# HJReachability/ilqgames

Measured on AMD Instinct MI355X. Metric: iLQ iterations/sec (batch), higher is better.
Workload: dtype f64

## Files before the change

### ilqgames_amd/csrc/ilqg_api.hip

```cpp
#include <hip/hip_runtime.h>

#include <cstdio>
#include <cstdlib>
#include <cmath>
#include <chrono>
#include <cstring>
#include <string>
#include <vector>

#include "ilqg_common.hpp"
#include "ilqg_lq.hpp"
#include "ilqg_lq_openloop.hpp"
#include "ilqg_lq_feedback2.hpp"
#include "ilqg_lq_generic.hpp"
#include "ilqg_costates.hpp"
#include "ilqg_models.hpp"
#include "ilqg_nash.hpp"
#include "ilqg_receding.hpp"
#include "ilqg_rowprog.hpp"
#include "ilqg_rowprog_static.hpp"
#include "ilqg_solve.hpp"
#include "ilqg_stages.hpp"

using namespace ilqg;
// ... 1366 lines not shown
  }
  const bool counted = !opt.forced_steps && (split || !(fixed_iters > 0 && !al_mode) || choice(opt.counted, false));
  const bool handoff = counted && !split && !kProfile && sa.prm.linesearch && choice(opt.handoff, true);
  const bool lists = split || handoff;
  sa.defer_forward = (!split && !open_loop) ? 1 : 0;
  {
    constexpr size_t fwd_elems = 4 * 2 * ((NX * NX + C::SCR + 3) & ~3) + 2 * NX + 8;
    if (trial_rows_elems(d, sa.rows_cw, static_prog != 0) < fwd_elems + 8) sa.defer_forward = 0;
  }
  const bool adjoint = choice(opt.adjoint_expected_decrease, sa.defer_forward == 0);
  const bool single_wave = has_1w && pw && sa.compact && !kProfile && (adjoint || sa.defer_forward) &&
                           d.rp_compact_w <= W1Cfg<T, NX, NP, MU>::kWords &&
                           choice(opt.single_wave_sweep, !opt.deterministic && size_t(sched_batch) >= size_t(5) * num_cus);
  if (single_wave) {
    sa.prio_div = 0;
    if (adjoint) sa.defer_forward = 0;
  }
  constexpr bool has_packed = sizeof(T) == 4 && C::USE_MFMA && C::MFMA_ONE_TILE && NP == 3;
  bool b_const = false;
  if (open_loop) {
    plan.sweep = {ol_compact ? ilq_lq_kernel<T, NX, NP, MU, LQ_OPEN_LOOP_COMPACT> : ilq_lq_kernel<T, NX, NP, MU, LQ_OPEN_LOOP>,
                  O::NT, (O::LDS_ELEMS + 4) * sizeof(T)};
  } else if constexpr (!C::USE_MFMA) {
    plan.sweep = {ilq_lq_kernel<T, NX, NP, MU, LQ_VALU_FEEDBACK>, C::NT, C::LDS_ELEMS * sizeof(T)};
  } else {
    plan.sweep = {ilq_lq_kernel<T, NX, NP, MU, LQ_PLAYER_WAVES>, 64 * NP,
                  (MfmaSweepLds<T, NX, NP, MU>::ELEMS + (C::MFMA_ONE_TILE ? 0 : 4)) * sizeof(T)};
    constexpr bool has_forms = C::MFMA_ONE_TILE && SolveRows<NP * MU, NX + 1>::FITS;
    const bool forms = choice(opt.sweep_forms, true);
    constexpr bool has_bconst = has_forms && NX < 16 && MU == 2;
    b_const = has_bconst && forms && p->b_constant && sa.compact && sa.defer_forward && !single_wave;
    if constexpr (has_forms)
      if (!forms) plan.sweep.kernel = ilq_lq_kernel<T, NX, NP, MU, LQ_PLAYER_WAVES, 0>;
    if constexpr (has_bconst)
      if (b_const) plan.sweep.kernel = ilq_lq_kernel<T, NX, NP, MU, LQ_PLAYER_WAVES, 2>;
    if constexpr (has_packed) {
      if (size_t(sched_batch) >= size_t(5) * 256) {
        plan.sweep.kernel = ilq_lq_kernel<T, NX, NP, MU, LQ_PLAYER_WAVES_PACKED>;
        if constexpr (has_forms)
          if (!forms) plan.sweep.kernel = ilq_lq_kernel<T, NX, NP, MU, LQ_PLAYER_WAVES_PACKED, 0>;
        if constexpr (has_bconst)
          if (b_const) plan.sweep.kernel = ilq_lq_kernel<T, NX, NP, MU, LQ_PLAYER_WAVES_PACKED, 2>;
      }
    }
    if constexpr (has_1w) {
      if (single_wave) {
        plan.sweep = {ilq_lq_kernel<T, NX, NP, MU, LQ_SINGLE_WAVE>, 64, size_t(W1Cfg<T, NX, NP, MU>::ELEMS + 4) * sizeof(T)};
        if constexpr (has_forms)
          if (!forms) plan.sweep.kernel = ilq_lq_kernel<T, NX, NP, MU, LQ_SINGLE_WAVE, 0>;
      }
    }
  }
  sa.clear_counters = 1;
  plan.trial = {k_trial, 64 * W, lds_trial};
  plan.exit = {ilq_exit_kernel<T, NX, NP, MU>, nt_exit, quad_tables_bytes(d, sizeof(T)) + 64 * sizeof(T)};
  plan.read_restarts = counted && al_mode;
  constexpr bool pairs = rollout_pairs(NX, NP, MU);
  if (lists) {
    const size_t lds_roll = trial_phase_lds_bytes<T>(d, TRIAL_ROLL, sa.rows_cw);
    const size_t lds_proll = pairs ? size_t(rollout_pair_lds_elems(d.n, d.m)) * sizeof(T) + 16 : lds_roll;
    const size_t static_regs_lds = (rows_state_in_registers(NX, NP * MU) ? 0 : size_t(d.n + d.m) * 64) * sizeof(T) + 16;
    const int rows_cw = static_id ? 64 : sa.rows_cw;
    const bool regs = static_id && static_in_regs;
    plan.roll = {ilq_roll_kernel<T, NX, NP, MU>, 64, lds_proll};
    plan.rows = {k_rows, 64, regs ? static_regs_lds : split_maps_bytes + split_rows_elems(d, NX, rows_cw) * sizeof(T)};
    plan.decide = {d.inst_solver ? ilq_decide_kernel<T, NX, NP, MU, true> : ilq_decide_kernel<T, NX, NP, MU, false>, 64,
                   trial_phase_lds_bytes<T>(d, TRIAL_DECIDE, sa.rows_cw)};
    plan.prows = {k_prows, 64, regs ? static_regs_lds : split_maps_bytes + probe_rows_elems(d, NX, rows_cw) * sizeof(T)};
    plan.proll = {ilq_probe_roll_kernel<T, NX, NP, MU>, 64, lds_proll};
    plan.proll_fat = {ilq_probe_roll_kernel<T, NX, NP, MU, sizeof(T) == 8>, 64, lds_proll};
    if (pairs) {
      plan.proll_single = {ilq_probe_roll_kernel<T, NX, NP, MU, sizeof(T) == 8, true>, 64, lds_roll};
      plan.proll_lanes = {ilq_probe_roll_lanes_kernel<T, NX, NP, MU>, 64, size_t(rollout_lanes_lds_elems(d.n, d.m, d.N)) * sizeof(T) + 16};
    }
  }
  plan.cap = al_mode ? (long long)(sa.prm.max_solver_iters + 1) * (sa.prm.unconstrained_solver_max_iters + 2)
                     : (long long)sa.prm.max_solver_iters + 2;
  if (split || counted) plan.cap = (plan.cap + 2) * ((long long)sa.prm.max_backtracking_steps + 3);
  plan.row_chunks = (d.T + sa.rows_cw - 1) / sa.rows_cw;
  plan.lane_width = rollout_lanes_per_wave(NP > 0 ? NP : 1);
  plan.num_cus = num_cus;
  plan.split = split; plan.counted = counted; plan.handoff = handoff; plan.lists = lists; plan.pairs = pairs;
  plan.timed = opt.max_runtime > 0.0 && counted;
  plan.bursts = counted && !kProfile && !plan.timed && choice(opt.round_bursts, true);
  plan.probe = lists && sa.prm.linesearch && choice(opt.probe, true);
  plan.lanes_auto = NX <= 16;
  plan.deep_tails = true;
  p->last_schedule = (single_wave ? ILQG_SCHEDULE_SINGLE_WAVE_SWEEP : 0) | ((single_wave && adjoint) ? ILQG_SCHEDULE_ADJOINT_DECREASE : 0) |
                     (split ? ILQG_SCHEDULE_SPLIT_TRIAL : 0) | (sa.compact ? ILQG_SCHEDULE_COMPACT_ROWS : 0) |
                     (counted ? ILQG_SCHEDULE_COUNTED : 0) | (open_loop ? ILQG_SCHEDULE_OPEN_LOOP : 0) |
                     ((static_prog || (static_id && split)) ? ILQG_SCHEDULE_STATIC_ROWS : 0) |
                     (b_const ? ILQG_SCHEDULE_CONSTANT_B : 0);
  return run_rounds(p, sa, tail, plan, opt, stream);
}

#if defined(ILQG_PART_NX)
template struct DimsLaunch<float, ILQG_PART_NX, ILQG_PART_NP, ILQG_PART_MU>;
template struct DimsLaunch<double, ILQG_PART_NX, ILQG_PART_NP, ILQG_PART_MU>;
#else
#if defined(ILQG_SPLIT_BUILD)
#define X(NX_, NP_, MU_)                                   \
  extern template struct DimsLaunch<float, NX_, NP_, MU_>; \
  extern template struct DimsLaunch<double, NX_, NP_, MU_>;
ILQG_FOR_DIMS(X)
#undef X
#endif

// ... 1020 lines not shown
```

### ilqgames_amd/csrc/ilqg_rows.hpp

```cpp
#pragma once

#include <type_traits>
#include <utility>

#include "ilqg_common.hpp"
#include "ilqg_models.hpp"

#ifndef ILQG_ROWS_XREG
#define ILQG_ROWS_XREG 1
#endif
#ifndef ILQG_PROFILE2
#define ILQG_PROFILE2 0
#endif

namespace ilqg {

#pragma clang fp contract(off)

typedef const __attribute__((address_space(4))) int* rp_cptr;
template <typename T> struct ConstPtr;
template <> struct ConstPtr<float> { typedef const __attribute__((address_space(4))) float* type; };
template <> struct ConstPtr<double> { typedef const __attribute__((address_space(4))) double* type; };

enum {
// ... 410 lines not shown
    if constexpr (BOUND && (F == RO_WEIGHT || F == RO_VALUE) && (mode == ROP_TERM || mode == ROP_EXT_EVAL || mode == ROP_EXT_APPLY || mode == ROP_JACOBIAN)) {
      const int c = cols[F == RO_WEIGHT ? 0 : 1];
      if (c >= 0 && iv) return iv[c];
    }
    return rt[F];
  }
  __device__ __forceinline__ SidsStatic<S, OP> sids() const { return SidsStatic<S, OP>{}; }
};
struct PassDynamic {
  int op_begin, op_end, reg_begin, reg_end, li_begin, li_count, pkind, player, li_grad;
};
template <class S, int PS>
struct PassStatic {
  static constexpr int b = S::w[RP_OFF_PASS] + PS * RPASS_WORDS;
  static constexpr int op_begin = S::w[b + 0], op_end = S::w[b + 1], reg_begin = S::w[b + 2], reg_end = S::w[b + 3],
                       li_begin = S::w[b + 4], li_count = S::w[b + 5], pkind = S::w[b + 6], player = S::w[b + 7],
                       li_grad = S::w[b + 8];
};

template <class S>
constexpr bool static_prog_in_registers() {
  const int nops = (S::w[RP_OFF_SIDS] - S::w[RP_OFF_OPS]) / ROP_WORDS;
  for (int op = 0; op < nops; op++) {
    const int b = S::w[RP_OFF_OPS] + op * ROP_WORDS;
    if (S::w[b + RO_MODE] == ROP_AFFINE || S::w[b + RO_NSID] > ROP_INLINE_SIDS) return false;
  }
  return S::w[RP_NUM_PSLOTS] + S::w[RP_MAX_LSLOTS] <= 64 && S::w[S::w[RP_OFF_COMPACT] + RC_W] > 0;
}
template <class S>
constexpr unsigned static_prog_pass_split() {
  const int np = S::w[RP_NUM_PASSES];
  int wgt[32] = {0};
  for (int ps = 0; ps < np && ps < 32; ps++) {
    const int b = S::w[RP_OFF_PASS] + ps * RPASS_WORDS;
    wgt[ps] = S::w[b + 1] - S::w[b + 0];
  }
  unsigned first = 0, taken = 0;
  int wa = 0, wb = 0;
  for (int k = 0; k < np && k < 32; k++) {
    int best = -1;
    for (int ps = 0; ps < np && ps < 32; ps++)
      if (!((taken >> ps) & 1u) && (best < 0 || wgt[ps] > wgt[best])) best = ps;
    taken |= 1u << best;
    if (wa <= wb) { first |= 1u << best; wa += wgt[best]; } else { wb += wgt[best]; }
  }
  return first;
}
template <class PROG, bool ST = PROG::STATIC> struct ProgInRegisters { static constexpr bool value = false; static constexpr int slots = 1; };
template <class PROG> struct ProgInRegisters<PROG, true> {
  static constexpr bool value = static_prog_in_registers<typename PROG::S>();
  static constexpr int slots = value ? PROG::S::w[RP_NUM_PSLOTS] + PROG::S::w[RP_MAX_LSLOTS] : 1;
};

template <typename T, int CN_, int CM_, int CNP_, bool XREG = false, bool GRAD_ONLY = false, class PROG = ProgDynamic>
__device__ __forceinline__ void rows_chunk(const DevProblem& p, const short* maps, const QuadArgs<T>& a, int k0,
                                           int nrows, int cw, T* sm, int lane, unsigned pass_mask = ~0u) {
  constexpr bool RT = CN_ == 0;
  constexpr bool ST = PROG::STATIC;
  static_assert(!XREG || (CN_ > 0 && CN_ <= 16 && CM_ <= 16), "register-held rows: compile-time n, m <= 16");
  const int CN = RT ? p.n : CN_, CM = RT ? p.m : CM_, CNP = RT ? p.N : CNP_;
  const int NA = CN + CM;
  constexpr bool REGACC = ProgInRegisters<PROG>::value;
  const int cws = REGACC ? 1 : (ST ? kStaticRowStride : cw + 1);
  const int ast = ST ? 64 : cw;
  T* const arg = sm;
  T* const acc = sm + (XREG ? 0 : NA) * ast;
  typedef typename std::conditional<XREG, MixArg<T>, RowArg<T>>::type Arg;
  const rp_cptr rp = (rp_cptr)p.row_prog;
  const rp_cptr iv = (rp_cptr) reinterpret_cast<const int*>(a.iv);
  const typename ConstPtr<T>::type segs =
      (typename ConstPtr<T>::type)(PROG::kBound ? problem_segs<T>(p) + a.seg_off : problem_segs<T>(p));
  auto hdr = [&](auto f) -> int {
    if constexpr (ST) { constexpr int v = PROG::S::w[decltype(f)::value]; return v; } else return rp[decltype(f)::value];
  };
#define ILQG_RP_HDR(F) hdr(std::integral_constant<int, F>{})
  const int num_passes = ILQG_RP_HDR(RP_NUM_PASSES), NPS = ILQG_RP_HDR(RP_NUM_PSLOTS);
  const rp_cptr passes = rp + ILQG_RP_HDR(RP_OFF_PASS);
  const rp_cptr ops = rp + ILQG_RP_HDR(RP_OFF_OPS);
  const rp_cptr sids = rp + ILQG_RP_HDR(RP_OFF_SIDS);
  const rp_cptr pinit = rp + ILQG_RP_HDR(RP_OFF_PINIT);
  const rp_cptr linit = rp + ILQG_RP_HDR(RP_OFF_LINIT);
  const rp_cptr regions = rp + ILQG_RP_HDR(RP_OFF_REGIONS);
  const rp_cptr merit = rp + ILQG_RP_HDR(RP_OFF_MERIT);
  const bool quad_out = !GRAD_ONLY && (a.Q != nullptr || (a.compact != nullptr && a.compact_quad));
  const bool do_quad = quad_out || a.merit_part != nullptr;
  const bool want_cost = !GRAD_ONLY && a.cost_part != nullptr;
  const PairTable& pt = p.pairs;
  long long qc0 = (kProfile && a.phacc) ? clock64() : 0, qc1;
#define ILQG_QPH(i) do { if (kProfile && a.phacc) { __builtin_amdgcn_sched_barrier(0); qc1 = clock64(); __builtin_amdgcn_sched_barrier(0); a.phacc[i] += qc1 - qc0; qc0 = qc1; } } while (0)

  {
    auto stage_rows = [&](const T* g, int dim, int first) {
      constexpr int UN = 8;
      const int total = cw * dim;
      for (int i0 = 0; i0 < total; i0 += 64 * UN) {
        T v[UN];
        int dst[UN];
#pragma unroll
        for (int u = 0; u < UN; u++) {
          const int i = i0 + u * 64 + lane;
          const bool in = i < total;
          const int ic = in ? i : 0;
          const int r = ic / dim, e = ic - r * dim;
          const int rs = r < nrows ? r : nrows - 1;
          dst[u] = in ? (first + e) * ast + r : -1;
          v[u] = g[rs * dim + e];
        }
// ... 184 lines not shown
        term_compute_leaf<T, Arg, true>(QuadTables<T>{}, c, v, lambda, a.mu, &o, &cc, tnom);
#if ILQG_PROFILE2
        ILQG_QPH(3);
#endif
        bool act = deriv && o.pattern != PAT_NONE;
        if (mode == ROP_EXT_EVAL) {
          const bool is_min = c.flags & ILQG_FLAG_IS_MIN;
          if (aux == 0 || (is_min && o.value < ext_value) || (!is_min && o.value > ext_value)) {
            ext_value = o.value;
            ext_best = aux;
          }
          return;
        }
        if (mode == ROP_EXT_APPLY) {
          if (aux == 0 && is_cost && live) ctot += ext_value;
          act = act && ext_best == aux;
        } else if (is_cost && live) {
          ctot += o.value;
        }
        if (act) {
          if (sid_inline)
            rows_scatter<T>(od.template field<RO_PATTERN_NSEG>(), o, sid, nsid, col, cws, v, quad_out);
          else
            rows_scatter<T>(od.template field<RO_PATTERN_NSEG>(), o, SidsTable{sids + od.template field<RO_SID>()}, nsid, col, cws, v, quad_out);
        }
#if ILQG_PROFILE2
        ILQG_QPH(4);
#endif
      };
      if constexpr (ST) {
        static_for<PD::op_begin, PD::op_end>([&](auto opc) {
          constexpr int OP = decltype(opc)::value;
          run_op(OpStatic<typename PROG::S, OP, PROG::kBound>{ops + OP * ROP_WORDS, iv, rp + (PROG::S::w[RP_WORDS] + OP * 2)});
        });
      } else {
        static_assert(ROP_WORDS <= 64, "an op descriptor is one word per lane");
        const int* const opsv = reinterpret_cast<const int*>(p.row_prog) + rp[RP_OFF_OPS];
        int next_words = (lane < ROP_WORDS && op_begin < op_end) ? opsv[op_begin * ROP_WORDS + lane] : 0;
#pragma unroll 1
        for (int op = op_begin; op < op_end; op++) {
          int words = next_words;
          if (op + 1 < op_end) next_words = lane < ROP_WORDS ? opsv[(op + 1) * ROP_WORDS + lane] : 0;
          if (iv) {
            const rp_cptr icols = rp + rp[RP_WORDS];
            const int wcol = icols[2 * op], vcol = icols[2 * op + 1];
            if (wcol >= 0) words = lane == RO_WEIGHT ? iv[wcol] : words;
            if (vcol >= 0) words = lane == RO_VALUE ? iv[vcol] : words;
          }
          run_op(OpDynamic{words});
        }
      }
      if (pkind == RPASS_PLAYER && valid) {
        if (want_cost) a.cost_part[size_t(row) * CNP + player] = ctot;
        if (a.merit_part) {
          T s1 = T(0), s2 = T(0);
          if constexpr (ST) {
            typedef typename PROG::S S;
            constexpr int mb = S::w[RP_OFF_MERIT] + PD::player * RMERIT_WORDS, sb = S::w[RP_OFF_SIDS];
            static_for<0, S::w[mb + 3]>([&](auto dc) {
              const T rv = col[S::w[sb + S::w[mb + 2] + decltype(dc)::value] * cws];
              s1 += rv * rv;
            });
            static_for<0, S::w[mb + 1]>([&](auto dc) {
              const T lv = col[S::w[sb + S::w[mb + 0] + decltype(dc)::value] * cws];
              s2 += lv * lv;
            });
          } else {
            const rp_cptr md = merit + player * RMERIT_WORDS;
            const rp_cptr ls = sids + md[0];
            const rp_cptr rs = sids + md[2];
            const int lcnt = md[1], rcnt = md[3];
            for (int d = 0; d < rcnt; d++) {
              const T rv = col[rs[d] * cws];
              s1 += rv * rv;
            }
            for (int d = 0; d < lcnt; d++) {
              const T lv = col[ls[d] * cws];
              s2 += lv * lv;
            }
          }
          a.merit_part[(size_t(row) * CNP + player) * 2 + 0] = s1;
          a.merit_part[(size_t(row) * CNP + player) * 2 + 1] = s2;
        }
      }
    }
    lds_sync(true);
    tl_stamp(a.tl, a.tl_b, 42 + 2 * (ps < 4 ? ps : 4), lane == 0);
#if !ILQG_PROFILE2
    if (pkind == RPASS_JACOBIANS) ILQG_QPH(1); else ILQG_QPH(2);
#else
    ILQG_QPH(0);
#endif
    if constexpr (!REGACC)
    for (int rg = reg_begin; rg < (GRAD_ONLY ? reg_begin : reg_end); rg++) {
      const rp_cptr rd = regions + rg * RREG_WORDS;
      const int arr = rd[0], words = rd[1], offs = rd[2];
      const short* const map = maps + rd[3];
      if (arr == RA_A) {
        if (a.A) {
          if constexpr (RT) rows_writeout_rt<T>(a.A + size_t(k0) * CN * CN, size_t(CN) * CN, CN * CN, map, acc, cws, nrows, lane);
          else rows_writeout<T, CN_ * CN_, rows_vec_width<T>(CN_ * CN_)>(a.A + size_t(k0) * CN * CN, CN * CN, map, acc, cws, nrows, lane);
        }
      } else if (arr == RA_B) {
        if (a.Bm) {
          if constexpr (RT) rows_writeout_rt<T>(a.Bm + size_t(k0) * CN * CM, size_t(CN) * CM, CN * CM, map, acc, cws, nrows, lane);
          else rows_writeout<T, CN_ * CM_, rows_vec_width<T>(CN_ * CM_)>(a.Bm + size_t(k0) * CN * CM, CN * CM, map, acc, cws, nrows, lane);
        }
      } else if (arr == RA_Q) {
        if (a.Q) {
          if constexpr (RT) rows_writeout_rt<T>(a.Q + size_t(k0) * CNP * CN * CN + offs, size_t(CNP) * CN * CN, CN * CN, map, acc, cws, nrows, lane);
          else rows_writeout<T, CN_ * CN_, rows_vec_width<T>(CN_ * CN_)>(a.Q + size_t(k0) * CNP * CN * CN + offs, size_t(CNP) * CN * CN, map, acc, cws, nrows, lane);
        }
      } else if (arr == RA_L) {
        if (a.l) rows_writeout_small<T>(a.l + size_t(k0) * CNP * CN + offs, CNP * CN, words, map, acc, cws, nrows, lane);
      } else if (arr == RA_R) {
        if (a.R) rows_writeout_small<T>(a.R + size_t(k0) * pt.Rsz + offs, pt.Rsz, words, map, acc, cws, nrows, lane);
      } else {
        if (a.r) rows_writeout_small<T>(a.r + size_t(k0) * pt.rsz + offs, pt.rsz, words, map, acc, cws, nrows, lane);
      }
    }
    if (!GRAD_ONLY && a.compact && (pkind == RPASS_PLAYER ? a.compact_quad : a.compact_lin)) {
      int CWD, base;
      if constexpr (ST) {
        typedef typename PROG::S S;
        constexpr int cbo = S::w[RP_OFF_COMPACT];
        CWD = S::w[cbo + RC_W];
        base = S::w[cbo + RC_BASE + (PD::pkind == RPASS_PLAYER ? 1 + PD::player : 0)];
      } else {
        const rp_cptr cb = rp + rp[RP_OFF_COMPACT];
        CWD = cb[RC_W];
        base = cb[RC_BASE + (pkind == RPASS_PLAYER ? 1 + player : 0)];
      }
      T* const g0 = a.compact + size_t(k0) * CWD + base;
      constexpr int RB = 8;
      if constexpr (REGACC) {
// ... 72 lines not shown
```

### ilqgames_amd/csrc/ilqg_solve.hpp

```cpp
#pragma once
#ifndef ILQG_ROLL_PRIO
#define ILQG_ROLL_PRIO 1
#endif

#include "ilqg_lq.hpp"
#include "ilqg_lq_openloop.hpp"
#include "ilqg_lq_feedback2.hpp"
#include "ilqg_lq_feedback1w.hpp"
#include "ilqg_lq_generic.hpp"
#include "ilqg_stages.hpp"

namespace ilqg {

template <typename T>
struct SolveArgs {
  const T* x0;
  T *xs, *us;
  T *P, *alpha;
  T* total_costs;
  int *iters, *status, *converged;
  const int* active;
  T* ws;
  size_t ws_stride;
  int fixed_iters;
  int batch;
  int ol_row;
  int al_mode;
  ilqg_solver_params prm;
  long long* prof;
  int first;
  int* unfinished;
  const int* ids;
  int* ids_next;
  int round_count;
  const T* forced_steps;
  int defer_forward;
  int prio_div;
  int compact;
  int rows_cw;
  T* probe_pool;
  int probe_k;
  int outer_closed;
  int clear_counters;
};


enum { ST_ROLLOUT = 0, ST_QUAD = 1, ST_LQ = 2, ST_INNER_DONE = 3, ST_DONE = 4, ST_PROBE = 5 };
enum { Q_COSTS = 0, Q_INIT = 1, Q_TRIAL = 2, Q_LIN = 3 };
template <typename T>
struct SolveState {
  int stage, qmode, initial, cur, sacc, num_iterations, bt, accepted_iters;
  int has_converged, ok, logged, inner_calls, al_success;
  int ed_pending;
  int rejected;
  int pad2;
  T acc_scale, step, last_merit, expected_decrease, max_err, mu;
};
constexpr int kStateElems = 32;
static_assert(sizeof(SolveState<float>) <= kStateElems * sizeof(float), "state slot");
static_assert(sizeof(SolveState<double>) <= kStateElems * sizeof(double), "state slot");

struct WsLayout {
  size_t xs1, us1, P1, al1, A, B, Q, l, R, r, lqscr, dx, mpart, cpart, ints, state, lambdas, wxs, wus, wP, wal, total;
  __host__ __device__ WsLayout(int n, int m, int N, int T, int Rsz, int rsz, int ol_row = 0, int num_constraints = 0,
                               int al_mode = 0) {
    size_t o = 0;
    auto take = [&](size_t cnt) {
      const size_t at = o;
      o += (cnt + 3) & ~size_t(3);
      return at;
    };
    xs1 = take(size_t(T) * n);
    us1 = take(size_t(T) * m);
    P1 = take(size_t(T) * m * n);
    al1 = take(size_t(T) * m);
    A = take(size_t(T) * n * n);
    B = take(size_t(T) * n * m);
    Q = take(size_t(T) * N * n * n);
    l = take(size_t(T) * N * n);
    R = take(size_t(T) * Rsz);
    r = take(size_t(T) * rsz);
    lqscr = take(size_t(T) * (size_t(ol_row) > size_t(N * (n + 1) + n) ? size_t(ol_row) : size_t(N * (n + 1) + n)));
    dx = take(size_t(T) * n);
    mpart = take(size_t(T) * N * 2);
    cpart = take(size_t(T) * N);
    ints = take(2 * kMaxPlayers);
    state = take(kStateElems);
    lambdas = take(size_t(num_constraints) * T);
    wxs = take(al_mode ? size_t(T) * n : 0);
    wus = take(al_mode ? size_t(T) * m : 0);
    wP = take(al_mode ? size_t(T) * m * n : 0);
    wal = take(al_mode ? size_t(T) * m : 0);
    total = o;
  }
};

// ... 544 lines not shown

template <typename T>
__device__ __forceinline__ void trial_rollout_args(const SolveArgs<T>& sa, const InstanceBuffers<T>& ib, int b, int n,
                                                   SolveState<T>& s, RolloutArgs<T>& ra) {
  const int snew = 1 - s.sacc;
  ra.x0 = s.initial ? sa.x0 + size_t(b) * n : ib.XS(s.cur);
  ra.xs_ref = s.initial ? ib.XS(0) : ib.XS(s.cur);
  ra.us_ref = s.initial ? ib.US(0) : ib.US(s.cur);
  ra.P = s.initial ? ib.PB(0) : ib.PB(snew);
  ra.alpha = s.initial ? ib.AL(0) : ib.AL(snew);
  ra.alpha_scale = s.initial ? T(1) : s.step;
  ra.xs = s.initial ? ib.XS(1) : ib.XS(1 - s.cur);
  ra.us = s.initial ? ib.US(1) : ib.US(1 - s.cur);
  if (s.initial) {
    s.cur = 1;
    s.qmode = Q_COSTS;
  } else {
    s.qmode = sa.prm.linesearch ? Q_TRIAL : Q_LIN;
  }
}

template <typename T, int NX, int NP, int MU>
__device__ __forceinline__ void roll_pair_instances(const DevProblem& p, const SolveArgs<T>& sa, int b0, int b1, T* sm) {
  constexpr int n = NX, N = NP, m = NP * MU;
  const InstanceBuffers<T> ib0(p, sa, b0), ib1(p, sa, b1 < 0 ? b0 : b1);
  SolveState<T> s0, s1;
  RolloutArgs<T> r0, r1;
  auto enter = [&](const InstanceBuffers<T>& ib, int b, SolveState<T>& s, RolloutArgs<T>& r) -> bool {
    if (b < 0) return false;
    if (!sa.first) {
      if (reinterpret_cast<const SolveState<T>*>(ib.w + ib.L.state)->stage != ST_ROLLOUT) return false;
    } else if (sa.active && !sa.active[b]) {
      if (threadIdx.x == 0) reinterpret_cast<SolveState<T>*>(ib.w + ib.L.state)->stage = ST_DONE;
      return false;
    }
    s = trial_state_begin<T>(p, sa, ib, b, n, N, m);
    if (s.stage != ST_ROLLOUT) return false;
    trial_rollout_args<T>(sa, ib, b, n, s, r);
    r.iv = instance_values(p, b);
    return true;
  };
  const bool g0 = enter(ib0, b0, s0, r0), g1 = enter(ib1, b1, s1, r1);
  if (!g0 && !g1) return;
  __syncthreads();
  rollout_pair<T, NX, NP * MU, (MU == 1)>(p, g0 ? r0 : r1, g1 ? r1 : r0, g0, g1, sm, int(threadIdx.x));
  if (g0) state_store<T>(ib0.w, ib0.L, s0);
  if (g1) state_store<T>(ib1.w, ib1.L, s1);
}

__host__ __device__ constexpr bool fused_rollout_room(int elem_bytes, int nx, int np, int mu, int progid) {
  return elem_bytes == 4 || (progid != 0 && nx == 14 && np == 3 && mu == 2);
}

template <typename T, int NX, int NP, int MU, int W, int PHASE = TRIAL_FUSED, int PROGID = 0, bool BOUND = (PROGID >= kBoundProg),
          bool SOLVER_COLS = true>
__device__ __forceinline__ void trial_part_instance(const DevProblem& p, const short* maps,
                                                    const SolveArgs<T>& sa, int b, T* sm) {
  static_assert(PHASE == TRIAL_FUSED || W == 1, "the split phases run one wave per instance");
  static_assert(NX > 0 || PHASE != TRIAL_FUSED, "the run-time-dimensioned path (NX = 0) runs the split passes");
  const int n = NX > 0 ? NX : p.n, N = NX > 0 ? NP : p.N, m = NX > 0 ? NP * MU : p.m;
  const int Tn = p.T;
  const InstanceBuffers<T> ib(p, sa, b);
  const WsLayout& L = ib.L;
  T* const w = ib.w;
  int* const t_extreme = ib.t_extreme();
  T* const lambdas = w + L.lambdas;
  T* const costs = sa.total_costs + size_t(b) * N;
  const int t = threadIdx.x, wave = t >> 6, lane = t & 63;

  const size_t re = PHASE == TRIAL_DECIDE ? 0 : (rollout_lds_elems(n, m) + 3) & ~size_t(3);
  const size_t qe = trial_phase_quad_elems<T>(p, PHASE, sa.rows_cw, PROGID != 0 && PHASE == TRIAL_FUSED);
  constexpr int RW = W > 1 ? W - 1 : 1;
  const int rwave = W > 1 ? wave - 1 : 0;
  T* const sm_roll = sm;
  T* const sm_quad = sm + re + size_t(rwave < 0 ? 0 : rwave) * qe;
  T* const sm_quad0 = sm + re;
  int* const flags = reinterpret_cast<int*>(sm + re + size_t(RW) * qe);
  T* const ed_slot = reinterpret_cast<T*>(flags + 2);

  SolveState<T> s = trial_state_begin<T>(p, sa, ib, b, n, N, m);
  tl_stamp(sa.prof, b, 0, t == 0);
  const long long pr_start = clock64();
  long long qph[8] = {0, 0, 0, 0, 0, 0, 0, 0};
  long long rph[4] = {0, 0, 0, 0};

#pragma unroll 1
  while (s.stage == ST_ROLLOUT || s.stage == ST_QUAD) {
    __syncthreads();
    const bool roll = PHASE != TRIAL_DECIDE && s.stage == ST_ROLLOUT;
    RolloutArgs<T> ra;
    if (roll) {
      trial_rollout_args<T>(sa, ib, b, n, s, ra);
      if constexpr (BOUND || PHASE == TRIAL_ROLL) ra.iv = instance_values(p, b);
    }
    if (t == 0) {
      flags[0] = roll ? 0 : Tn;
      flags[1] = 0;
    }
    __syncthreads();
    tl_stamp(sa.prof, b, 1, t == 0);
    if (roll && wave == 0) {
#if ILQG_ROLL_PRIO
      __builtin_amdgcn_s_setprio(ILQG_ROLL_PRIO);
#endif
      if constexpr (NX > 0)
        rollout_instance<T, NX, NP * MU, (NX == 4 && NP == 2), (MU == 1), (NX == 3 && NP == 2 && MU == 1),
                         (NX == 4 * NP && MU == 2 && NP <= 2), dims_use_plain_rk4(NX, NP, MU),
                         fused_rollout_room(int(sizeof(T)), NX, NP, MU, PROGID)>(
                                         p, ra, sm_roll, lane, W > 1 ? &flags[0] : nullptr,
                                         (kProfile && sa.prof) ? rph : nullptr, kTimeline ? sa.prof : nullptr, b);
      else
        rollout_instance_rt<T>(p, ra, sm_roll, lane);
#if ILQG_ROLL_PRIO
      __builtin_amdgcn_s_setprio(0);
#endif
    }
    tl_stamp(sa.prof, b, 2, t == 0);
    if (roll && W == 1) {
      __syncthreads();
      if (t == 0) flags[0] = Tn;
      __syncthreads();
    }
    if (PHASE == TRIAL_ROLL) break;

    const int qmode = s.qmode;
    if constexpr (PHASE == TRIAL_FUSED) {
    QuadArgs<T> qa = trial_quad_args<T, BOUND>(p, ib, s, sa.compact != 0, b);
    qa.phacc = (kProfile && sa.prof) ? qph : nullptr;
    qa.tl = kTimeline ? sa.prof : nullptr;
    qa.tl_b = b;
    long long tq0 = (kProfile && sa.prof) ? clock64() : 0;
    static_assert(W <= 2, "the deferred forward pass reads the linearisation on the first row wave while no other row wave "
                          "may overwrite it yet: with more than one row wave set defer_forward = 0 or hold them back");
    if (s.ed_pending && rwave == 0) {
      LQArgs<T> fa{};
      fa.A = w + L.A;
      fa.scratch = w + L.lqscr;
      fa.x0 = nullptr;
      fa.dx = nullptr;
      fa.ed_out = ed_slot;
      fa.T_steps = Tn;
      if (sa.compact) {
        fa.compact = w + L.Q;
        fa.compact_tab = p.row_prog + p.rp_compact_off;
        fa.dt = p.dt;
      }
      constexpr int FWD_LDSE = 4 * 2 * ((NX * NX + LQCfg<T, NX, NP, MU>::SCR + 3) & ~3) + 2 * NX + 8;
      lq_forward_pass_body<T, NX, NP, MU, 64, FWD_LDSE>(fa, sm_quad, lane);
    }
    tl_stamp(sa.prof, b, 3, rwave == 0 && lane == 0);
    typedef typename RowProgSel<PROGID>::type RowProg;
    constexpr bool SHARE_LAST = PROGID != 0 && W == 2 && ProgInRegisters<RowProg>::value && rows_state_in_registers(NX, NP * MU);
    if constexpr (SHARE_LAST) {
      const int cw = sa.rows_cw;
      const int nchunks = (Tn + cw - 1) / cw;
      const int rem = Tn % cw;
      constexpr unsigned first_half = static_prog_pass_split<typename RowProg::S>();
      if (wave == 0) qa.tl = nullptr;
#pragma unroll 1
      for (int c = (wave == 0 ? nchunks - 1 : 0); c < nchunks; c++) {
        const int k0 = rem == 0 ? c * cw : (c == 0 ? 0 : rem + (c - 1) * cw);
        const int nrows = (rem != 0 && c == 0) ? rem : cw;
        if (wave != 0)
          while (progress_observe(&flags[0]) < k0 + nrows) __builtin_amdgcn_s_sleep(8);
        tl_stamp(sa.prof, b, 4 + 2 * (c < 3 ? c : 3), wave != 0 && lane == 0);
        const unsigned mask = c == nchunks - 1 ? (wave == 0 ? first_half : ~first_half) : ~0u;
        rows_chunk<T, NX, NP * MU, NP, true, false, RowProg>(p, maps, qa, k0, nrows, cw, sm_quad, lane, mask);
        tl_stamp(sa.prof, b, 5 + 2 * (c < 3 ? c : 3), wave != 0 && lane == 0);
      }
    } else
    if (rwave >= 0) {
      const int cw = sa.rows_cw;
      const int nchunks = (Tn + cw - 1) / cw;
      auto claim = [&]() {
        int c = 0;
        if (lane == 0) c = atomicAdd(&flags[1], 1);
        return __builtin_amdgcn_readfirstlane(c);
      };
      const int rem = Tn % cw;
#pragma unroll 1
      for (int c = claim(); c < nchunks; c = claim()) {
        const int k0 = rem == 0 ? c * cw : (c == 0 ? 0 : rem + (c - 1) * cw);
        const int nrows = (rem != 0 && c == 0) ? rem : cw;
        while (progress_observe(&flags[0]) < k0 + nrows) __builtin_amdgcn_s_sleep(8);
        if (kProfile && sa.prof) { const long long tq1 = clock64(); qph[6] += tq1 - tq0; }
        tl_stamp(sa.prof, b, 4 + 2 * (c < 3 ? c : 3), lane == 0);
        rows_chunk<T, NX, NP * MU, NP, (PROGID != 0 && rows_state_in_registers(NX, NP * MU)), false, typename RowProgSel<PROGID>::type>(
            p, maps, qa, k0, nrows, cw, sm_quad, lane);
        tl_stamp(sa.prof, b, 5 + 2 * (c < 3 ? c : 3), lane == 0);
        if (kProfile && sa.prof) { tq0 = clock64(); qph[7] += 1; }
      }
    }
    }

    if (PHASE == TRIAL_FUSED && s.ed_pending) {
      __syncthreads();
      s.expected_decrease = uniform(*ed_slot);
      s.ed_pending = 0;
      __syncthreads();
    }
    tl_stamp(sa.prof, b, 12, t == 0);
    ilqg_solver_params prm = sa.prm;
    if constexpr (SOLVER_COLS) prm = solver_params_of(p, sa.prm, b);
    const int max_iters = solve_max_iters(sa, prm);
    if (qmode == Q_COSTS) {
      costs_reduce<T>(p, w + L.cpart, costs, t_extreme, sm_quad0, int(qe));
      s.qmode = Q_INIT;
      s.stage = ST_QUAD;
    } else if (qmode == Q_INIT) {
      s.initial = 0;
      s.stage = (s.num_iterations < max_iters) ? ST_LQ : ST_INNER_DONE;
    } else {
      bool accepted = true;
      bool costs_ready = false;
      if (qmode == Q_TRIAL) {
        T merit_v = T(0);
        costs_ready = merit_costs_reduce<T>(p, w + L.mpart, w + L.cpart, t_extreme, sm_quad0, int(qe), &merit_v);
        const T merit = costs_ready ? uniform(merit_v) : uniform(merit_reduce<T>(p, w + L.mpart, sm_quad0, int(qe)));
        tl_stamp(sa.prof, b, 14, t == 0);
        const T scaled = T(prm.expected_decrease_fraction) * s.step * s.expected_decrease;
        accepted = (s.last_merit - merit >= scaled) || sa.forced_steps != nullptr;
        if (accepted) {
          const T diff = s.last_merit - merit;
          s.has_converged =
              (merit <= s.last_merit) && ((diff < T(0) ? -diff : diff) < T(prm.convergence_tolerance));
          s.last_merit = merit;
        }
      } else {
        __syncthreads();
      }
      if (accepted) {
        s.cur = 1 - s.cur;
        s.sacc = 1 - s.sacc;
        s.acc_scale = s.step;
        s.accepted_iters++;
        if (costs_ready)
          costs_commit<T>(p, sm_quad0, costs, t_extreme);
        else
          costs_reduce<T>(p, w + L.cpart, costs, t_extreme, sm_quad0, int(qe));
        s.stage = (s.num_iterations < max_iters && (sa.fixed_iters > 0 || !s.has_converged)) ? ST_LQ : ST_INNER_DONE;
      } else {
        s.bt++;
        s.rejected++;
        if (s.bt >= prm.max_backtracking_steps) {
          s.ok = 0;
          s.stage = ST_INNER_DONE;
        } else {
          s.step *= T(prm.geometric_alpha_scaling);
          s.stage = ST_ROLLOUT;
        }
      }
    }
    tl_stamp(sa.prof, b, 15, t == 0);
    if (PHASE == TRIAL_DECIDE) break;
    if (PHASE == TRIAL_FUSED && sa.ids_next != nullptr && s.stage == ST_ROLLOUT && s.bt > 0) break;
  }
  state_store<T>(w, L, s);
  tl_stamp(sa.prof, b, 13, t == 0);
  if (PHASE == TRIAL_ROLL) return;
  if (t == 0) {
    const int slot = s.stage == ST_LQ ? 0 : (s.stage == ST_ROLLOUT || s.stage == ST_QUAD) ? 3 : 1;
    const int at = atomicAdd(sa.unfinished + slot, 1);
    if (slot == 3 && sa.ids_next) sa.ids_next[at] = b;
  }
  if (kProfile && t == 0 && sa.prof) sa.prof[size_t(b) * 96 + 1] += clock64() - pr_start;
  if (kProfile && t == 0 && sa.prof) {
#pragma unroll
    for (int i = 0; i < 4; i++) sa.prof[size_t(b) * 96 + 88 + i] += rph[i];
  }
  if (kProfile && lane == 0 && sa.prof && wave < 2) {
#pragma unroll
    for (int i = 0; i < 8; i++) sa.prof[size_t(b) * 96 + 64 + 8 * wave + i] += qph[i];
  }
}

template <typename T>
struct IterLog {
  T *xs, *us, *costs, *P, *alpha;
  int* count;
  int capacity;
};

template <typename T>
__device__ __forceinline__ void log_part_instance(const DevProblem& p, const SolveArgs<T>& sa, const IterLog<T>& lg, int b) {
  const InstanceBuffers<T> ib(p, sa, b);
  const SolveState<T> s = state_load<T>(ib.w, ib.L);
  if (s.stage != ST_LQ && s.stage != ST_INNER_DONE) return;
  const int slot = (sa.al_mode ? s.logged : 0) + s.accepted_iters;
  const int t = threadIdx.x, nt = blockDim.x;
// ... 160 lines not shown
```

### ilqgames_amd/csrc/ilqg_stages.hpp

```cpp
#pragma once

#include "ilqg_common.hpp"
#include "ilqg_models.hpp"

#ifndef ILQG_ROLLOUT_PAIRS
#define ILQG_ROLLOUT_PAIRS 1
#endif

namespace ilqg {

template <typename T>
struct RolloutArgs {
  const T* x0;
  const T* xs_ref;
  const T* us_ref;
  const T* P;
  const T* alpha;
  T alpha_scale;
  T* xs;
  T* us;
  const float* iv = nullptr;
};

__host__ __device__ inline int rollout_stage_elems(int n, int m) { return (m * n + 2 * m + n + 3) & ~3; }
// ... 399 lines not shown
    lc[LC_SREG + t] = __float_as_int(p.state_reg[t]);
    lc[LC_CREG + t] = __float_as_int(p.control_reg[t]);
    lc[LC_STRUCT + t] = p.structure[t];
    lc[LC_PII + t] = p.pairs.pii[t];
  }
  if (t <= kMaxPlayers) {
    lc[LC_XOFF + t] = p.xoff[t];
    lc[LC_UOFF + t] = p.uoff[t];
  }
  if (t < kMaxPairs) {
    lc[LC_PI + t] = p.pairs.pi[t];
    lc[LC_PJ + t] = p.pairs.pj[t];
    lc[LC_ROFF + t] = p.pairs.roff[t];
    lc[LC_RGOFF + t] = p.pairs.rgoff[t];
    lc[LC_FROMCOST + t] = p.pairs.from_cost[t];
  }
  __syncthreads();
  if (const float* iv = instance_values(p, inst)) {
    constexpr int TW = int(sizeof(DevTerm) / sizeof(int));
    for (int c = t; c < p.inst_count; c += NT) {
      const int term = p.inst_terms[2 * c], field = p.inst_terms[2 * c + 1];
      if (term < 0) continue;
      const int word = int((field == ILQG_PARAM_WEIGHT ? offsetof(DevTerm, weight) : offsetof(DevTerm, value)) / sizeof(int));
      terms_i[term * TW + word] = __float_as_int(iv[c]);
    }
    __syncthreads();
  }
  QuadTables<T> tb;
  tb.terms = reinterpret_cast<const DevTerm*>(terms_i);
  tb.segs = segs;
  tb.poly_off = poff;
  tb.order = order;
  tb.lc = lc;
  tb.tnom = problem_time_nominal<T>(p) + instance_tnom_offset(p, inst);
  tb.tnom_T = p.T;
  tb.dense = problem_dense<T>(p);
  return tb;
}

template <typename T>
struct QuadArgs {
  const T* xs;
  const T* us;
  const T* lambdas;
  T mu;
  const int* t_extreme;
  double t_init;
  T *A, *Bm;
  T *Q, *l, *R, *r;
  T* compact = nullptr;
  bool compact_lin = false, compact_quad = false;
  T* merit_part;
  T* cost_part;
  const float* iv = nullptr;
  size_t seg_off = 0;
  size_t tnom_off = 0;
  long long* phacc = nullptr;
  long long* tl = nullptr;
  int tl_b = 0;
};

template <typename T>
__device__ __forceinline__ void stage_to_lds(T* sm, const T* g, int count) {
  constexpr int UN = 8;
  const int nt = blockDim.x;
  for (int e0 = threadIdx.x; e0 < count; e0 += nt * UN) {
    T v[UN];
#pragma unroll
    for (int u = 0; u < UN; u++) {
      const int e = e0 + u * nt;
      v[u] = g[e < count ? e : e0];
    }
#pragma unroll
    for (int u = 0; u < UN; u++) {
      const int e = e0 + u * nt;
      if (e < count) sm[e] = v[u];
    }
  }
}

template <typename T, typename F>
__device__ __forceinline__ void lds_ordered_visit(const T* v, int count, F&& visit) {
  constexpr int U = 8;
  int e = 0;
  if (count >= U) {
    T x[U];
#pragma unroll
    for (int u = 0; u < U; u++) x[u] = v[u];
    for (; e + 2 * U <= count; e += U) {
      T y[U];
#pragma unroll
      for (int u = 0; u < U; u++) y[u] = v[e + U + u];
#pragma unroll
      for (int u = 0; u < U; u++) visit(e + u, x[u]);
#pragma unroll
      for (int u = 0; u < U; u++) x[u] = y[u];
    }
#pragma unroll
    for (int u = 0; u < U; u++) visit(e + u, x[u]);
    e += U;
  }
  for (; e < count; e++) visit(e, v[e]);
}

template <typename T>
__device__ __forceinline__ T merit_reduce(const DevProblem& p, const T* merit_part, T* sm, int sm_elems = 0) {
  __syncthreads();
  const int count = p.T * p.N * 2;
  if (count + 1 <= sm_elems) {
    stage_to_lds<T>(sm, merit_part, count);
    __syncthreads();
    if (threadIdx.x == 0) {
      T merit = T(0);
      const int skip = p.N * 2;
      for (int e = 0; e < skip && e < count; e += 2) merit += sm[e];
      lds_ordered_visit<T>(sm + skip, count - skip, [&](int, T x) { merit += x; });
      sm[count] = T(0.5) * merit;
    }
    __syncthreads();
    const T v = sm[count];
    __syncthreads();
    return v;
  }
  if (threadIdx.x == 0) {
    T merit = T(0);
    for (int k = 0; k < p.T; k++)
      for (int i = 0; i < p.N; i++) {
        merit += merit_part[(size_t(k) * p.N + i) * 2 + 0];
        if (k > 0) merit += merit_part[(size_t(k) * p.N + i) * 2 + 1];
      }
    sm[0] = T(0.5) * merit;
  }
  __syncthreads();
  const T v = sm[0];
  __syncthreads();
  return v;
}

template <typename T>
__device__ __forceinline__ bool merit_costs_reduce(const DevProblem& p, const T* merit_part, const T* cost_part,
                                                   const int* t_extreme, T* sm, int sm_elems, T* merit_out) {
  const int cm = p.T * p.N * 2, cc = p.T * p.N;
  if (cm + cc + 2 * kMaxPlayers + 4 > sm_elems) return false;
  __syncthreads();
  T* const smc = sm + cm;
  T* const res = smc + cc;
  stage_to_lds<T>(sm, merit_part, cm);
  stage_to_lds<T>(smc, cost_part, cc);
  __syncthreads();
  const int cw0 = blockDim.x > 64 ? 64 : 0;
  if (threadIdx.x == 0) {
    T merit = T(0);
    const int skip = p.N * 2;
    for (int e = 0; e < skip && e < cm; e += 2) merit += sm[e];
    lds_ordered_visit<T>(sm + skip, cm - skip, [&](int, T x) { merit += x; });
    res[0] = T(0.5) * merit;
  }
  const int i = int(threadIdx.x) - cw0;
  if (i >= 0 && i < p.N) {
    const int st = p.structure[i];
    T c = st == ILQG_SUM ? T(0) : (st == ILQG_MAX ? -dinf<T>() : dinf<T>());
    int te = t_extreme ? t_extreme[i] : 0;
    auto visit = [&](int k, T v) {
      if (st == ILQG_SUM)
        c += v;
      else if (st == ILQG_MAX && v > c) {
        c = v;
        te = k;
      } else if (st == ILQG_MIN && v < c) {
        c = v;
        te = k;
      }
    };
    int k = 0;
    for (; k + 8 <= p.T; k += 8) {
      T x[8];
#pragma unroll
      for (int u = 0; u < 8; u++) x[u] = smc[(k + u) * p.N + i];
#pragma unroll
      for (int u = 0; u < 8; u++) visit(k + u, x[u]);
    }
    for (; k < p.T; k++) visit(k, smc[k * p.N + i]);
    res[1 + i] = c;
    res[1 + kMaxPlayers + i] = T(te);
  }
  __syncthreads();
  *merit_out = res[0];
  return true;
}
template <typename T>
__device__ __forceinline__ void costs_commit(const DevProblem& p, const T* sm, T* costs_out, int* t_extreme) {
  const T* const res = sm + p.T * p.N * 3;
  const int i = threadIdx.x;
  if (i < p.N) {
    costs_out[i] = res[1 + i];
    if (t_extreme) t_extreme[i] = int(res[1 + kMaxPlayers + i]);
  }
  __syncthreads();
}

template <typename T>
__device__ __forceinline__ void costs_reduce(const DevProblem& p, const T* cost_part, T* costs_out, int* t_extreme,
                                             T* sm = nullptr, int sm_elems = 0) {
  __syncthreads();
  const int i = threadIdx.x;
  const int count = p.T * p.N;
  const bool staged = sm != nullptr && count <= sm_elems;
  if (staged) {
    stage_to_lds<T>(sm, cost_part, count);
    __syncthreads();
  }
  if (i < p.N) {
    const int st = p.structure[i];
    T c = st == ILQG_SUM ? T(0) : (st == ILQG_MAX ? -dinf<T>() : dinf<T>());
    int te = t_extreme ? t_extreme[i] : 0;
    auto visit = [&](int k, T v) {
      if (st == ILQG_SUM)
        c += v;
      else if (st == ILQG_MAX && v > c) {
        c = v;
        te = k;
      } else if (st == ILQG_MIN && v < c) {
        c = v;
        te = k;
      }
    };
    if (staged) {
      int k = 0;
      for (; k + 8 <= p.T; k += 8) {
        T x[8];
#pragma unroll
        for (int u = 0; u < 8; u++) x[u] = sm[(k + u) * p.N + i];
#pragma unroll
        for (int u = 0; u < 8; u++) visit(k + u, x[u]);
      }
      for (; k < p.T; k++) visit(k, sm[k * p.N + i]);
    } else {
      for (int k = 0; k < p.T; k++) visit(k, cost_part[size_t(k) * p.N + i]);
    }
    costs_out[i] = c;
    if (t_extreme) t_extreme[i] = te;
  }
  __syncthreads();
}

}

#include "ilqg_rows.hpp"
```

Before: 2.204 million.

## Accumulate trial merit and cost partials in LDS incrementally during row chunks

For the fused trial kernel with a static row program in registers and two waves, the row evaluation also writes per-row merit and cost partials into a reserved LDS region. Threads then fold each finished chunk into running sums while later chunks are still being computed. At the end only the last chunk needs reducing, so the global-memory staging and the full serial reduction after the rows are avoided. It also switches chunking to short-last-chunk ordering, relaxes one barrier into lds_sync, and needs extra LDS, which is only granted when four blocks still fit in 160 KB.

```diff
diff --git a/ilqgames_amd/csrc/ilqg_api.hip b/ilqgames_amd/csrc/ilqg_api.hip
--- a/ilqgames_amd/csrc/ilqg_api.hip
+++ b/ilqgames_amd/csrc/ilqg_api.hip
@@ -1442,7 +1442,13 @@
     }
   }
   sa.clear_counters = 1;
-  plan.trial = {k_trial, 64 * W, lds_trial};
+  size_t lds_part_bytes = 0;
+  if (static_prog && static_in_regs && W == 2 && fused_partials_room(int(sizeof(T)), NX, NP, MU)) {
+    const size_t extra = partials_lds_elems(d.T, d.N) * sizeof(T);
+    if (4 * (lds_trial + extra) <= size_t(160) * 1024) lds_part_bytes = extra;
+  }
+  sa.lds_part = lds_part_bytes ? 1 : 0;
+  plan.trial = {k_trial, 64 * W, lds_trial + lds_part_bytes};
   plan.exit = {ilq_exit_kernel<T, NX, NP, MU>, nt_exit, quad_tables_bytes(d, sizeof(T)) + 64 * sizeof(T)};
   plan.read_restarts = counted && al_mode;
   constexpr bool pairs = rollout_pairs(NX, NP, MU);
diff --git a/ilqgames_amd/csrc/ilqg_rows.hpp b/ilqgames_amd/csrc/ilqg_rows.hpp
--- a/ilqgames_amd/csrc/ilqg_rows.hpp
+++ b/ilqgames_amd/csrc/ilqg_rows.hpp
@@ -486,7 +486,8 @@
   static constexpr int slots = value ? PROG::S::w[RP_NUM_PSLOTS] + PROG::S::w[RP_MAX_LSLOTS] : 1;
 };
 
-template <typename T, int CN_, int CM_, int CNP_, bool XREG = false, bool GRAD_ONLY = false, class PROG = ProgDynamic>
+template <typename T, int CN_, int CM_, int CNP_, bool XREG = false, bool GRAD_ONLY = false, class PROG = ProgDynamic,
+          bool LDSP = false>
 __device__ __forceinline__ void rows_chunk(const DevProblem& p, const short* maps, const QuadArgs<T>& a, int k0,
                                            int nrows, int cw, T* sm, int lane, unsigned pass_mask = ~0u) {
   constexpr bool RT = CN_ == 0;
@@ -777,6 +778,8 @@
       }
       if (pkind == RPASS_PLAYER && valid) {
         if (want_cost) a.cost_part[size_t(row) * CNP + player] = ctot;
+        if constexpr (LDSP)
+          if (want_cost && a.lds_cost) a.lds_cost[row * CNP + player] = ctot;
         if (a.merit_part) {
           T s1 = T(0), s2 = T(0);
           if constexpr (ST) {
@@ -806,6 +809,11 @@
           }
           a.merit_part[(size_t(row) * CNP + player) * 2 + 0] = s1;
           a.merit_part[(size_t(row) * CNP + player) * 2 + 1] = s2;
+          if constexpr (LDSP)
+            if (a.lds_merit) {
+              a.lds_merit[(row * CNP + player) * 2 + 0] = s1;
+              a.lds_merit[(row * CNP + player) * 2 + 1] = s2;
+            }
         }
       }
     }
diff --git a/ilqgames_amd/csrc/ilqg_solve.hpp b/ilqgames_amd/csrc/ilqg_solve.hpp
--- a/ilqgames_amd/csrc/ilqg_solve.hpp
+++ b/ilqgames_amd/csrc/ilqg_solve.hpp
@@ -42,6 +42,7 @@
   int probe_k;
   int outer_closed;
   int clear_counters;
+  int lds_part;
 };
 
 
@@ -692,6 +693,18 @@
   return elem_bytes == 4 || (progid != 0 && nx == 14 && np == 3 && mu == 2);
 }
 
+__host__ __device__ constexpr bool fused_partials_room(int elem_bytes, int nx, int np, int mu) {
+  return elem_bytes == 4 || (nx == 14 && np == 3 && mu == 2);
+}
+
+#ifndef ILQG_SHORT_CHUNK_LAST
+#define ILQG_SHORT_CHUNK_LAST 1
+#endif
+__device__ __forceinline__ int trial_last_chunk_begin(int Tn, int cw) {
+  if (Tn <= cw) return 0;
+  return ILQG_SHORT_CHUNK_LAST ? ((Tn + cw - 1) / cw - 1) * cw : Tn - cw;
+}
+
 template <typename T, int NX, int NP, int MU, int W, int PHASE = TRIAL_FUSED, int PROGID = 0, bool BOUND = (PROGID >= kBoundProg),
           bool SOLVER_COLS = true>
 __device__ __forceinline__ void trial_part_instance(const DevProblem& p, const short* maps,
@@ -717,9 +730,13 @@
   T* const sm_quad0 = sm + re;
   int* const flags = reinterpret_cast<int*>(sm + re + size_t(RW) * qe);
   T* const ed_slot = reinterpret_cast<T*>(flags + 2);
+  T* const part_lds = reinterpret_cast<T*>(flags + 4);
 
   SolveState<T> s = trial_state_begin<T>(p, sa, ib, b, n, N, m);
   tl_stamp(sa.prof, b, 0, t == 0);
+  if (kTimeline && PHASE == TRIAL_FUSED && sa.prof && lane == 0 && wave < 2)
+    sa.prof[size_t(b) * 96 + 32 + 30 + wave] = (long long)__builtin_amdgcn_s_getreg((31 << 11) | 4) |
+                                               ((long long)__builtin_amdgcn_s_getreg((31 << 11) | 20) << 32);
   const long long pr_start = clock64();
   long long qph[8] = {0, 0, 0, 0, 0, 0, 0, 0};
   long long rph[4] = {0, 0, 0, 0};
@@ -764,8 +781,15 @@
     if (PHASE == TRIAL_ROLL) break;
 
     const int qmode = s.qmode;
+    constexpr bool LDS_RED = PHASE == TRIAL_FUSED && PROGID != 0 && W == 2 && fused_partials_room(int(sizeof(T)), NX, NP, MU) &&
+                             ProgInRegisters<typename RowProgSel<PROGID>::type>::value && rows_state_in_registers(NX, NP * MU);
+    const bool lds_red = LDS_RED && sa.lds_part != 0 && qmode == Q_TRIAL;
     if constexpr (PHASE == TRIAL_FUSED) {
     QuadArgs<T> qa = trial_quad_args<T, BOUND>(p, ib, s, sa.compact != 0, b);
+    if (lds_red) {
+      qa.lds_merit = part_lds;
+      qa.lds_cost = part_lds + size_t(Tn) * N * 2;
+    }
     qa.phacc = (kProfile && sa.prof) ? qph : nullptr;
     qa.tl = kTimeline ? sa.prof : nullptr;
     qa.tl_b = b;
@@ -799,14 +823,16 @@
       if (wave == 0) qa.tl = nullptr;
 #pragma unroll 1
       for (int c = (wave == 0 ? nchunks - 1 : 0); c < nchunks; c++) {
-        const int k0 = rem == 0 ? c * cw : (c == 0 ? 0 : rem + (c - 1) * cw);
-        const int nrows = (rem != 0 && c == 0) ? rem : cw;
+        constexpr bool SHORT_LAST = ILQG_SHORT_CHUNK_LAST && LDS_RED;
+        const int k0 = (SHORT_LAST || rem == 0) ? c * cw : (c == 0 ? 0 : rem + (c - 1) * cw);
+        const int nrows = SHORT_LAST ? (Tn - k0 < cw ? Tn - k0 : cw) : ((rem != 0 && c == 0) ? rem : cw);
         if (wave != 0)
           while (progress_observe(&flags[0]) < k0 + nrows) __builtin_amdgcn_s_sleep(8);
         tl_stamp(sa.prof, b, 4 + 2 * (c < 3 ? c : 3), wave != 0 && lane == 0);
         const unsigned mask = c == nchunks - 1 ? (wave == 0 ? first_half : ~first_half) : ~0u;
-        rows_chunk<T, NX, NP * MU, NP, true, false, RowProg>(p, maps, qa, k0, nrows, cw, sm_quad, lane, mask);
+        rows_chunk<T, NX, NP * MU, NP, true, false, RowProg, LDS_RED>(p, maps, qa, k0, nrows, cw, sm_quad, lane, mask);
         tl_stamp(sa.prof, b, 5 + 2 * (c < 3 ? c : 3), wave != 0 && lane == 0);
+        if (lds_red && c < nchunks - 1) partials_extend<T>(p, part_lds, t_extreme, k0, k0 + nrows, c == 0, 64, 65);
       }
     } else
     if (rwave >= 0) {
@@ -833,6 +859,13 @@
     }
     }
 
+    if (lds_red) {
+      lds_sync(false);
+      if (s.ed_pending) {
+        s.expected_decrease = uniform(*ed_slot);
+        s.ed_pending = 0;
+      }
+    } else
     if (PHASE == TRIAL_FUSED && s.ed_pending) {
       __syncthreads();
       s.expected_decrease = uniform(*ed_slot);
@@ -855,6 +888,12 @@
       bool costs_ready = false;
       if (qmode == Q_TRIAL) {
         T merit_v = T(0);
+        if (lds_red) {
+          partials_extend<T>(p, part_lds, t_extreme, trial_last_chunk_begin(Tn, sa.rows_cw), Tn, Tn <= sa.rows_cw, 0, 64);
+          lds_sync(false);
+          merit_v = T(0.5) * part_lds[size_t(Tn) * N * 3];
+          costs_ready = true;
+        } else
         costs_ready = merit_costs_reduce<T>(p, w + L.mpart, w + L.cpart, t_extreme, sm_quad0, int(qe), &merit_v);
         const T merit = costs_ready ? uniform(merit_v) : uniform(merit_reduce<T>(p, w + L.mpart, sm_quad0, int(qe)));
         tl_stamp(sa.prof, b, 14, t == 0);
@@ -874,7 +913,9 @@
         s.sacc = 1 - s.sacc;
         s.acc_scale = s.step;
         s.accepted_iters++;
-        if (costs_ready)
+        if (lds_red)
+          costs_commit<T, false>(p, part_lds, costs, t_extreme);
+        else if (costs_ready)
           costs_commit<T>(p, sm_quad0, costs, t_extreme);
         else
           costs_reduce<T>(p, w + L.cpart, costs, t_extreme, sm_quad0, int(qe));
diff --git a/ilqgames_amd/csrc/ilqg_stages.hpp b/ilqgames_amd/csrc/ilqg_stages.hpp
--- a/ilqgames_amd/csrc/ilqg_stages.hpp
+++ b/ilqgames_amd/csrc/ilqg_stages.hpp
@@ -475,6 +475,8 @@
   bool compact_lin = false, compact_quad = false;
   T* merit_part;
   T* cost_part;
+  T* lds_merit = nullptr;
+  T* lds_cost = nullptr;
   const float* iv = nullptr;
   size_t seg_off = 0;
   size_t tnom_off = 0;
@@ -518,6 +520,31 @@
       for (int u = 0; u < U; u++) visit(e + u, x[u]);
 #pragma unroll
       for (int u = 0; u < U; u++) x[u] = y[u];
+    }
+#pragma unroll
+    for (int u = 0; u < U; u++) visit(e + u, x[u]);
+    e += U;
+  }
+  for (; e < count; e++) visit(e, v[e]);
+}
+
+template <typename T, typename F>
+__device__ __forceinline__ void lds_ordered_visit2(const T* v, int count, F&& visit) {
+  constexpr int U = 8;
+  int e = 0;
+  if (count >= 2 * U) {
+    T x[U], y[U];
+#pragma unroll
+    for (int u = 0; u < U; u++) x[u] = v[u];
+    for (; e + 3 * U <= count; e += 2 * U) {
+#pragma unroll
+      for (int u = 0; u < U; u++) y[u] = v[e + U + u];
+#pragma unroll
+      for (int u = 0; u < U; u++) visit(e + u, x[u]);
+#pragma unroll
+      for (int u = 0; u < U; u++) x[u] = v[e + 2 * U + u];
+#pragma unroll
+      for (int u = 0; u < U; u++) visit(e + U + u, y[u]);
     }
 #pragma unroll
     for (int u = 0; u < U; u++) visit(e + u, x[u]);
@@ -611,7 +638,7 @@
   *merit_out = res[0];
   return true;
 }
-template <typename T>
+template <typename T, bool SYNC = true>
 __device__ __forceinline__ void costs_commit(const DevProblem& p, const T* sm, T* costs_out, int* t_extreme) {
   const T* const res = sm + p.T * p.N * 3;
   const int i = threadIdx.x;
@@ -619,7 +646,62 @@
     costs_out[i] = res[1 + i];
     if (t_extreme) t_extreme[i] = int(res[1 + kMaxPlayers + i]);
   }
-  __syncthreads();
+  if constexpr (SYNC) __syncthreads();
+}
+
+__host__ __device__ inline size_t partials_lds_elems(int T, int N) {
+  return (size_t(T) * N * 3 + 2 * kMaxPlayers + 4 + 3) & ~size_t(3);
+}
+template <typename T>
+__device__ __forceinline__ void partials_extend(const DevProblem& p, T* pl, const int* t_extreme, int k0, int k1,
+                                                bool first, int merit_thread, int cost_thread0) {
+  const int cm = p.T * p.N * 2, cc = p.T * p.N;
+  T* const smc = pl + cm;
+  T* const res = smc + cc;
+  if (int(threadIdx.x) == merit_thread) {
+    T merit = first ? T(0) : res[0];
+    int e0 = k0 * p.N * 2;
+    const int e1 = k1 * p.N * 2;
+    if (k0 == 0) {
+      const int skip = p.N * 2;
+      for (int e = 0; e < skip && e < e1; e += 2) merit += pl[e];
+      e0 = skip;
+    }
+    if (e1 > e0) lds_ordered_visit2<T>(pl + e0, e1 - e0, [&](int, T x) { merit += x; });
+    res[0] = merit;
+  }
+  const int i = int(threadIdx.x) - cost_thread0;
+  if (i >= 0 && i < p.N) {
+    const int st = p.structure[i];
+    T c = st == ILQG_SUM ? T(0) : (st == ILQG_MAX ? -dinf<T>() : dinf<T>());
+    int te = t_extreme ? t_extreme[i] : 0;
+    if (!first) {
+      c = res[1 + i];
+      te = int(res[1 + kMaxPlayers + i]);
+    }
+    auto visit = [&](int k, T v) {
+      if (st == ILQG_SUM)
+        c += v;
+      else if (st == ILQG_MAX && v > c) {
+        c = v;
+        te = k;
+      } else if (st == ILQG_MIN && v < c) {
+        c = v;
+        te = k;
+      }
+    };
+    int k = k0;
+    for (; k + 8 <= k1; k += 8) {
+      T x[8];
+#pragma unroll
+      for (int u = 0; u < 8; u++) x[u] = smc[(k + u) * p.N + i];
+#pragma unroll
+      for (int u = 0; u < 8; u++) visit(k + u, x[u]);
+    }
+    for (; k < k1; k++) visit(k, smc[k * p.N + i]);
+    res[1 + i] = c;
+    res[1 + kMaxPlayers + i] = T(te);
+  }
 }
 
 template <typename T>
```

New measurement: 2.245 million, median of 6. 1.8% higher.
